# elasota/ConvectionKernels

Measured on AMD Instinct MI355X. Metric: bc7_encode_default_plan_throughput, higher is better.
Workload: dtype f32+u16; 1 GPU; EncodeBC7, BC7EncodingPlan() + Options(), 4096x4096 SplitMix64 random RGBA, seed 2, 1048576 blocks resident in HBM (BASELINE configs[1]); blocks=1048576, exchange=none, search=exact branch-and-bound (output bit-identical)

## Files before the change

### convectionkernels_amd/api.py

```python
import ctypes
import functools
import os
import sys

import numpy as np

_HERE = os.path.dirname(os.path.abspath(__file__))
_LIB_PATH = os.path.join(_HERE, "lib", "libcvtt_mi355x.so")

NumParallelBlocks = 8


class Flags:
    BC7_FastIndexing = 0x008
    BC7_TrySingleColor = 0x010
    BC7_RespectPunchThrough = 0x020
    BC6H_FastIndexing = 0x040
    S3TC_Exhaustive = 0x080
    S3TC_Paranoid = 0x100
    Uniform = 0x200
    ETC_UseFakeBT709 = 0x400
    ETC_FakeBT709Accurate = 0x800
    Fastest = BC6H_FastIndexing | BC7_FastIndexing | S3TC_Paranoid
    Faster = Fastest
# ... 792 lines not shown
            n = b.size // bpb
            if b.size % bpb or n % NumParallelBlocks:
                raise CvttError("packed must hold a multiple of 8 %d-byte blocks" % bpb)
            shape, dt = self._decoded_layout(fmt, n)
            res = np.empty(shape, dt)
            with self._host_lock:
                self._check(self._lib.cvttmi_decode(self._h, fid, res.ctypes.data, b.ctypes.data, n), "decode(%s)" % fmt)
            return res
        import torch
        b = self._device_in(packed, "packed")
        nbytes = b.numel() * b.element_size()
        n = nbytes // bpb
        if nbytes % bpb or n % NumParallelBlocks:
            raise CvttError("packed must hold a multiple of 8 %d-byte blocks" % bpb)
        shape, dt = self._decoded_layout(fmt, n)
        res = torch.empty(shape, dtype={np.int16: torch.int16, np.int8: torch.int8, np.uint8: torch.uint8}[dt], device=b.device)
        stream = self._stream(stream, b.device)
        self._check(self._lib.cvttmi_decode_device(self._h, fid, res.data_ptr(), b.data_ptr(), n, ctypes.c_void_p(stream)),
                    "decode(%s)" % fmt)
        return res

    def measure_error(self, fmt, blocks, packed, per_block=False, stream=None):
        fid, bpb, tex, _ = self._texture_format(fmt)
        hdr = texel_class(fmt) == "half"
        if isinstance(packed, np.ndarray):
            b = np.ascontiguousarray(packed, np.uint8)
            s = np.ascontiguousarray(blocks)
            n = b.size // bpb
            if b.size % bpb or n % NumParallelBlocks or s.nbytes != n * tex:
                raise CvttError("packed must hold a multiple of 8 %d-byte blocks and blocks exactly as many %d-byte source blocks"
                                % (bpb, tex))
            totals = ErrorTotals()
            pb = np.empty(n, np.float32 if hdr else np.uint32) if per_block else None
            with self._host_lock:
                self._check(self._lib.cvttmi_measure_error(self._h, fid, b.ctypes.data, s.ctypes.data, n,
                                                           pb.ctypes.data if per_block else None, ctypes.addressof(totals)),
                            "measure_error(%s)" % fmt)
            return ErrorReport(fmt, totals, pb)
        import torch
        b = self._device_in(packed, "packed")
        s = self._device_in(blocks, "blocks")
        nbytes = b.numel() * b.element_size()
        n = nbytes // bpb
        if nbytes % bpb or n % NumParallelBlocks or s.numel() * s.element_size() != n * tex:
            raise CvttError("packed must hold a multiple of 8 %d-byte blocks and blocks exactly as many %d-byte source blocks"
                            % (bpb, tex))
        return self._measure_device(fmt, n, per_block, stream, b.device, lambda pb, tot, st: self._lib.cvttmi_measure_error_device(
            self._h, fid, b.data_ptr(), s.data_ptr(), n, pb, tot, st))

    def _measure_device(self, fmt, n, per_block, stream, device, call):
        import torch
        hdr = texel_class(fmt) == "half"
        tot = torch.empty(ctypes.sizeof(ErrorTotals), dtype=torch.uint8, device=device)
        pb = torch.empty(n, dtype=torch.float32 if hdr else torch.int32, device=device) if per_block else None
        stream = self._stream(stream, device)
        self._check(call(pb.data_ptr() if per_block else None, tot.data_ptr(), ctypes.c_void_p(stream)), "measure(%s)" % fmt)
        torch.cuda.synchronize(device)
        totals = ErrorTotals.from_buffer_copy(tot.cpu().numpy().tobytes())
        return ErrorReport(fmt, totals, pb)

    def measure_image(self, fmt, image, packed, per_block=False, stream=None):
        import torch
        fid, bpb, _, _ = self._texture_format(fmt)
        if not (isinstance(image, torch.Tensor) and image.is_cuda and image.dim() == 3 and image.shape[2] == 4):
            raise CvttError("image must be a CUDA tensor of shape (H, W, 4)")
        if image.device.index != self.device:
            raise CvttError("image lives on cuda:%d but this context was created for cuda:%d" % (image.device.index, self.device))
        if image.stride(2) != 1 or image.stride(1) != 4:
            image = image.contiguous()
        h, w = int(image.shape[0]), int(image.shape[1])
        esz = image.element_size()
        b = self._device_in(packed, "packed")
        n = ((w + 3) // 4) * ((h + 3) // 4)
        if b.numel() * b.element_size() != n * bpb:
            raise CvttError("packed must hold the %d blocks of a %dx%d image" % (n, w, h))
        return self._measure_device(fmt, n, per_block, stream, b.device, lambda pb, tot, st: self._lib.cvttmi_measure_image_error_device(
            self._h, fid, b.data_ptr(), image.data_ptr(), w, h, image.stride(0) * esz, 0 if esz == 1 else 1, pb, tot, st))

    def selftest_arith(self, count=1 << 22, seed=1):
        d, q = ctypes.c_uint64(0), ctypes.c_uint64(0)
        self._check(self._lib.cvttmi_selftest_arith(self._h, count, seed, ctypes.byref(d), ctypes.byref(q)), "selftest_arith")
        return int(d.value), int(q.value)

    def tile_image(self, image, stream=None):
        import torch
        image = self._image_in(image)
        h, w = int(image.shape[0]), int(image.shape[1])
        esz = image.element_size()
        n = self._lib.cvttmi_tiled_block_count(w, h)
        blocks = torch.empty((n, 16, 4), dtype=image.dtype, device=image.device)
        if stream is None:
            stream = torch.cuda.current_stream(image.device).cuda_stream
        self._check(self._lib.cvttmi_tile_image_device(self._h, blocks.data_ptr(), image.data_ptr(), w, h,
                                                       image.stride(0) * esz, 0 if esz == 1 else 1, ctypes.c_void_p(stream)), "tile_image")
        return blocks

    def compact_rows(self, packed, width, height, stream=None):
        import torch
        packed = self._device_in(packed, "packed")
        bpb = int(packed.shape[1])
        out = torch.empty((((height + 3) // 4) * ((width + 3) // 4), bpb), dtype=torch.uint8, device=packed.device)
        if stream is None:
            stream = torch.cuda.current_stream(packed.device).cuda_stream
        self._check(self._lib.cvttmi_compact_rows_device(self._h, out.data_ptr(), packed.contiguous().data_ptr(), width, height, bpb,
                                                         ctypes.c_void_p(stream)), "compact_rows")
        return out

    def encode_image(self, fmt, image, options=None, plan=None, stream=None):
        h, w = int(image.shape[0]), int(image.shape[1])
        blocks = self.tile_image(image, stream)
        if not has_image_form(fmt):
            raise CvttError("unknown format %r" % (fmt,))
        packed = self.encode(fmt, blocks, options, plan, stream=stream)
        return packed if w % 32 == 0 else self.compact_rows(packed, w, h, stream)

    def _image_in(self, image):
        import torch
        if not (isinstance(image, torch.Tensor) and image.is_cuda and image.dim() == 3 and image.shape[2] == 4):
            raise CvttError("image must be a CUDA tensor of shape (H, W, 4)")
        if image.device.index != self.device:
            raise CvttError("image lives on cuda:%d but this context was created for cuda:%d" % (image.device.index, self.device))
        if image.element_size() not in (1, 2):
            raise CvttError("image must be RGBA8 or RGBA16F")
        return image if image.stride(2) == 1 and image.stride(1) == 4 else image.contiguous()

    def _one_layer(self, image):
        image = self._image_in(image)
        if image.stride(0) < 4 * image.shape[1] or image.stride(0) % 4:
            raise CvttError("image rows must be whole texels and at least a row apart")
        return image[None]

    def build_mips(self, image, levels=None, signed=False, stream=None, filter="box", kernel=None, wrap="clamp"):
        return self.build_mips_array(self._one_layer(image), levels, signed, stream, filter, kernel, wrap)[0]

    def encode_mips(self, fmt, image, options=None, plan=None, levels=None, stream=None, mip_filter="box", kernel=None, wrap="clamp"):
        import torch
        if not has_image_form(fmt):
            raise CvttError("unknown format %r" % (fmt,))
        if isinstance(image, torch.Tensor) and image.dtype == torch.int8 and texel_class(fmt) != "snorm8":
            raise CvttError("%s is not encoded from an int8 image (bc4s / bc5s are)" % fmt)
        return self.encode_texture(fmt, self._one_layer(image), options, plan, levels, "layer", mip_filter, stream, kernel, wrap)[0]

    def _images_in(self, images):
        import torch
        if isinstance(images, (list, tuple)):
            images = [self._image_in(t) for t in images]
            if not images or any(t.shape != images[0].shape or t.dtype != images[0].dtype for t in images):
                raise CvttError("images must be a non-empty list of (H, W, 4) tensors of one size and dtype")
            images = torch.stack(images)
        if not (isinstance(images, torch.Tensor) and images.is_cuda and images.dim() == 4 and images.shape[3] == 4 and images.shape[0] >= 1
                and images.shape[1] >= 1 and images.shape[2] >= 1):
            raise CvttError("images must be a CUDA tensor of shape (L, H, W, 4) or a list of (H, W, 4) CUDA tensors")
        if images.device.index != self.device:
            raise CvttError("images live on cuda:%d but this context was created for cuda:%d" % (images.device.index, self.device))
        if images.element_size() not in (1, 2):
            raise CvttError("images must be RGBA8 or RGBA16F")
        n, h, w = (int(v) for v in images.shape[:3])
        row = images.stride(1) if h > 1 else 4 * w
        layer = images.stride(0) if n > 1 else h * row
        if not (images.stride(3) == 1 and images.stride(2) == 4 and row >= 4 * w and row % 4 == 0 and layer >= h * row and layer % 4 == 0):
            images = images.contiguous()
            row, layer = 4 * w, 4 * w * h
        esz = images.element_size()
        return images, row * esz, layer * esz

    def build_mips_array(self, images, levels=None, signed=False, stream=None, filter="box", kernel=None, wrap="clamp"):
# ... 354 lines not shown
```

### convectionkernels_amd/csrc/bc7_bounds.h

```cpp
#pragma once

namespace
{
typedef short v2s __attribute__((ext_vector_type(2)));

__device__ __forceinline__ int dot2(u32 a, u32 b, int acc)
{
    return __builtin_amdgcn_sdot2(__builtin_bit_cast(v2s, a), __builtin_bit_cast(v2s, b), acc, false);
}

__device__ __forceinline__ constexpr int tri(int r, int c) { return r >= c ? r * (r + 1) / 2 + c : c * (c + 1) / 2 + r; }

struct BlockScatter
{
    float S[10];
    float meanW[4];
};

__device__ __forceinline__ void blockRawSumsQuad(const u32 (&pix)[16], int c, int (&s)[4], int (&p)[10])
{
#pragma unroll
    for (int i = 0; i < 4; i++)
        s[i] = 0;
#pragma unroll
// ... 535 lines not shown
        P.tUU = dot2(P.U[k], P.U[k], P.tUU);
        P.tVV = dot2(P.V[k], P.V[k], P.tVV);
        P.tUV = dot2(P.U[k], P.V[k], P.tUV);
    }
    }
}

struct Sums2D
{
    int n, u, v, uu, vv, uv;
};

__device__ __forceinline__ void maskedSumsSel(const Proj2D<true> &P, int n, const uint4 &sel, Sums2D &m)
{
    m.n = n;
    m.u = m.v = m.uu = m.vv = m.uv = 0;
    const u32 s4[4] = {sel.x, sel.y, sel.z, sel.w};
#pragma unroll
    for (int k = 0; k < 4; k++)
    {
        const u32 um = P.U[k] & s4[k], vm = P.V[k] & s4[k];
        m.u = dot4s(um, 0x01010101u, m.u);
        m.v = dot4s(vm, 0x01010101u, m.v);
        m.uu = dot4s(um, P.U[k], m.uu);
        m.vv = dot4s(vm, P.V[k], m.vv);
        m.uv = dot4s(um, P.V[k], m.uv);
    }
}

template <bool G8>
__device__ __forceinline__ void maskedSums(const Proj2D<G8> &P, u32 mask, Sums2D &m)
{
    m.n = __popc(mask);
    m.u = m.v = m.uu = m.vv = m.uv = 0;
    if constexpr (G8)
    {
#pragma unroll
    for (int k = 0; k < 4; k++)
    {
        const u32 bits = (((mask >> (4 * k)) & 0xfu) * 0x00204081u) & 0x01010101u;
        const u32 sel = (bits << 8) - bits;
        const u32 um = P.U[k] & sel, vm = P.V[k] & sel;
        m.u = dot4s(um, 0x01010101u, m.u);
        m.v = dot4s(vm, 0x01010101u, m.v);
        m.uu = dot4s(um, P.U[k], m.uu);
        m.vv = dot4s(vm, P.V[k], m.vv);
        m.uv = dot4s(um, P.V[k], m.uv);
    }
    }
    else
    {
#pragma unroll
    for (int k = 0; k < 8; k++)
    {
        const u32 lo = (u32)__builtin_amdgcn_sbfe(mask, 2 * k, 1);
        const u32 hi = (u32)__builtin_amdgcn_sbfe(mask, 2 * k + 1, 1);
        const u32 sel = (lo & 0x0000ffffu) | (hi & 0xffff0000u);
        const u32 um = P.U[k] & sel, vm = P.V[k] & sel;
        m.u = dot2(um, 0x00010001u, m.u);
        m.v = dot2(vm, 0x00010001u, m.v);
        m.uu = dot2(um, P.U[k], m.uu);
        m.vv = dot2(vm, P.V[k], m.vv);
        m.uv = dot2(um, P.V[k], m.uv);
    }
    }
}

template <bool G8 = false>
__device__ __forceinline__ float subsetBound2D(const Sums2D &m, float rcpN, float invScaleSq, float twoDelta)
{
    const int a = (G8 ? __mul24(m.n, m.uu) : m.n * m.uu) - __mul24(m.u, m.u);
    const int c = (G8 ? __mul24(m.n, m.vv) : m.n * m.vv) - __mul24(m.v, m.v);
    const int b = (G8 ? __mul24(m.n, m.uv) : m.n * m.uv) - __mul24(m.u, m.v);
    const float fa = (float)a, fc = (float)c, fb = (float)b;
    const float half = (fa + fc) * 0.5f;
    const float diff = (fa - fc) * 0.5f;
    const float rad = __builtin_amdgcn_sqrtf(__fmaf_rn(diff, diff, fb * fb));
    const float lam = half * 0.999998f - rad * 1.000002f;
    const float L = fmaxf(lam, 0.0f) * invScaleSq;
    const float lb = (L * rcpN - twoDelta * __builtin_amdgcn_sqrtf(L)) * 0.9999f;
    return fmaxf(lb, 0.0f);
}

}

__device__ __forceinline__ u32 everyFourth(u64 m, int c)
{
    u64 x = (m >> c) & 0x1111111111111111ull;
    x = (x | (x >> 3)) & 0x0303030303030303ull;
    x = (x | (x >> 6)) & 0x000f000f000f000full;
    x = (x | (x >> 12)) & 0x000000ff000000ffull;
    x = (x | (x >> 24)) & 0xffffull;
    return (u32)x;
}
```

### convectionkernels_amd/csrc/bc7_kernel.hip

```cpp
#include <hip/hip_runtime.h>
#include <stdint.h>
#include <float.h>
#include <type_traits>
#include <stdlib.h>

#include "cvtt_device.h"

constexpr int kMaxPTRefine = 2;
constexpr float kBoundGrid16 = 2000.0f, kBoundLimit16 = 2040.0f;
constexpr float kBoundGrid8 = 124.0f, kBoundLimit8 = 127.0f;
#ifndef CVTT_GRID8_RGBA
#define CVTT_GRID8_RGBA true
#endif
#ifndef CVTT_GRID8_RGB
#define CVTT_GRID8_RGB true
#endif
#ifndef CVTT_BC7_WAVES
#define CVTT_BC7_WAVES 4
#endif
#ifndef CVTT_BC7_WAVES_SLOW
#define CVTT_BC7_WAVES_SLOW 4
#endif
#ifndef CVTT_EIG_ITERS
#define CVTT_EIG_ITERS 6
// ... 41 lines not shown
#define PROF_STAGE_LANES(stage, slot, pred) { const unsigned long long v_ = (unsigned long long)__popcll(__ballot(pred)); if (threadIdx.x == 0 && v_) atomicAdd(&g_bc7Stage[stage][slot], v_); }
#define PROF_STAGE2(stage, slot, n) { const unsigned long long v_ = (unsigned long long)(n); if (threadIdx.x == 0 && v_) atomicAdd(&g_bc7Stage2[stage][slot], v_); }
extern "C" int cvttmi_bc7_dup_read(unsigned long long *out)
{
    unsigned long long zero[8] = {0};
    if (hipMemcpyFromSymbol(out, HIP_SYMBOL(g_bc7Dup), sizeof(zero)) != hipSuccess) return -1;
    if (hipMemcpyToSymbol(HIP_SYMBOL(g_bc7Dup), zero, sizeof(zero)) != hipSuccess) return -1;
    return 0;
}
#define PROF_DECL unsigned long long profT = __builtin_readcyclecounter(); unsigned long long profAcc[16] = {0, 0, 0, 0, 0, 0, 0, 0, 0, 0, 0, 0, 0, 0, 0, 0}; unsigned long long profCnt[8] = {0, 0, 0, 0, 0, 0, 0, 0};
#define PROF_MARK(slot) { const unsigned long long now = __builtin_readcyclecounter(); profAcc[slot] += now - profT; profT = now; }
#define PROF_FLUSH if (threadIdx.x == 0) { unsigned long long tot = 0; for (int i = 0; i < 16; i++) { atomicAdd(&g_bc7Prof[i], profAcc[i]); tot += profAcc[i]; } \
    int bucket = 63 - __builtin_clzll(tot | 1ull) - 12; bucket = bucket < 0 ? 0 : (bucket > 15 ? 15 : bucket); atomicAdd(&g_bc7Prof[16 + bucket], 1ull); \
    } { unsigned long long wsum[8]; for (int i = 0; i < 8; i++) { unsigned long long v = profCnt[i]; if (i >= 4) { for (int st = 1; st < 64; st <<= 1) v += __shfl_xor(v, st); } wsum[i] = v; } \
    if (threadIdx.x == 0) { for (int i = 0; i < 8; i++) atomicAdd(&g_bc7Prof[32 + i], wsum[i]); \
    const unsigned long long passes = profCnt[2] / 64ull; int pb = 63 - __builtin_clzll(passes | 1ull); pb = pb > 7 ? 7 : pb; atomicAdd(&g_bc7Prof[40 + pb], 1ull); } }
#define PROF_COUNT(slot, n) { profCnt[slot] += (unsigned long long)(n); }
extern "C" int cvttmi_bc7_prof_read(unsigned long long *out)
{
    unsigned long long zero[48] = {0};
    if (hipMemcpyFromSymbol(out, HIP_SYMBOL(g_bc7Prof), sizeof(zero)) != hipSuccess) return -1;
    if (hipMemcpyToSymbol(HIP_SYMBOL(g_bc7Prof), zero, sizeof(zero)) != hipSuccess) return -1;
    return 0;
}
#else
#define PROF_DECL
#define PROF_MARK(slot)
#define PROF_COUNT(slot, n)
#define PROF_FLUSH
#define PROF_STAGE(stage, slot, n)
#define PROF_STAGE2(stage, slot, n)
#define PROF_STAGE_LANES(stage, slot, pred)
#endif

#ifdef CVTT_BC7_BOUND_DUMP
__device__ u32 *g_bc7BoundBuf;
__device__ u32 g_bc7BoundCap;
__device__ u32 g_bc7BoundCount;
extern "C" int cvttmi_bc7_bound_dump_set(void *deviceBuffer, uint32_t capacityRecords)
{
    const uint32_t zero = 0;
    u32 *buf = static_cast<u32 *>(deviceBuffer);
    if (hipMemcpyToSymbol(HIP_SYMBOL(g_bc7BoundBuf), &buf, sizeof(buf)) != hipSuccess) return -1;
    if (hipMemcpyToSymbol(HIP_SYMBOL(g_bc7BoundCap), &capacityRecords, sizeof(capacityRecords)) != hipSuccess) return -1;
    if (hipMemcpyToSymbol(HIP_SYMBOL(g_bc7BoundCount), &zero, sizeof(zero)) != hipSuccess) return -1;
    return 0;
}
extern "C" int cvttmi_bc7_bound_dump_count(uint32_t *out)
{
    return hipMemcpyFromSymbol(out, HIP_SYMBOL(g_bc7BoundCount), sizeof(*out)) == hipSuccess ? 0 : -1;
}
enum : u32 { BD_WHOLE6 = 0, BD_ROT = 1, BD_TIER1 = 2, BD_FULL = 3, BD_SHARP = 4, BD_PROBE_FULL = 5, BD_PROBE_SHARP = 6, BD_FINAL = 7 };
enum : u32 { BD_FORM = 0, BD_FORM_CMP = 1, BD_RELOAD = 2, BD_SUBSET = 3, BD_END = 4 };
__device__ __noinline__ void boundDumpEmit(u32 block, u32 w1, u32 w2, u32 w3, float computed, float stored, float err, u32 dropped,
                                           float x0, float x1, float x2, float x3)
{
    u32 *const buf = g_bc7BoundBuf;
    if (buf == nullptr)
        return;
    const u32 at = atomicAdd(&g_bc7BoundCount, 1u);
    if (at >= g_bc7BoundCap)
        return;
    u32 *r = buf + (size_t)at * 12u;
    r[0] = block;
    r[1] = w1;
    r[2] = w2;
    r[3] = w3;
    r[4] = __builtin_bit_cast(u32, computed);
    r[5] = __builtin_bit_cast(u32, stored);
    r[6] = __builtin_bit_cast(u32, err);
    r[7] = dropped;
    r[8] = __builtin_bit_cast(u32, x0);
    r[9] = __builtin_bit_cast(u32, x1);
    r[10] = __builtin_bit_cast(u32, x2);
    r[11] = __builtin_bit_cast(u32, x3);
}
#define BOUND_DUMP(...) do { __VA_ARGS__; } while (0)
#else
#define BOUND_DUMP(...)
#endif

#include "bc7_chain.h"
#include "bc7_dual.h"
#include "bc7_bounds.h"

template <bool FAST, bool PT, bool HARD>
__device__ __forceinline__ void bc7Body(const uint8_t *__restrict__ blocks, uint8_t *__restrict__ out,
                                        const CvttBc7Args &A, const CvttDeviceTables *__restrict__ T,
                                        const CvttBc7DevicePlan *__restrict__ dplan, const u32 vBlock, const u32 vGrid)
{
    __shared__ unsigned short s_bound[64][16];
    auto lbLoadRaw = [&](int partition, int b) -> float { return __builtin_bit_cast(float, (u32)s_bound[partition][b] << 16); };
    auto lbLoad = [&](int partition, int b) -> float { return __builtin_fabsf(lbLoadRaw(partition, b)); };
    auto lbStore = [&](int partition, int b, float v) { s_bound[partition][b] = (unsigned short)(__builtin_bit_cast(u32, v) >> 16); };
    auto lbStoreTier2 = [&](int partition, int b, float v) { s_bound[partition][b] = (unsigned short)((__builtin_bit_cast(u32, v) >> 16) | 0x8000u); };
    u32 *const s_raw = reinterpret_cast<u32 *>(&s_bound[0][0]);
    __shared__ u32 s_pix[16][16];
    __shared__ u32 s_blkFlags[16];
    __shared__ int s_scatter[16][14];
    __shared__ u32 s_item[64];
    __shared__ uint8_t s_myItems[PT ? 16 : 1][32];
    __shared__ UnitRec s_unit[64];
    __shared__ u32 s_parked[16][2];
    __shared__ float s_static[16];
    __shared__ unsigned short s_pm2[64];
    __shared__ u32 s_pm3[64];
    __shared__ __attribute__((aligned(16))) u32 s_res[64][5];
    __shared__ float s_trialErr[PT ? 32 * 16 * kMaxPTRefine : 1];
    float *const trialHbm = (PT && A.ptTrial) ? A.ptTrial + (size_t)vBlock * (size_t)(32 * 16) * (size_t)(A.refineRounds < 1 ? 1 : A.refineRounds) : nullptr;
    const cvttmi_bc7_plan *__restrict__ plan = &dplan->plan;
    int lane = threadIdx.x;
    int c = lane & 3;
    int blk = lane >> 2;
#define REFRESH_LANE() do { lane = (int)__builtin_amdgcn_mbcnt_hi(~0u, __builtin_amdgcn_mbcnt_lo(~0u, 0u)); asm volatile("" : "+v"(lane)); c = lane & 3; blk = lane >> 2; } while (0)
    u32 hardIndex = 0, hardBlock = 0;
    u64 hardMine = 0;
    float hardErr = FLT_MAX;
    int hardSeq = -1;
    if (HARD)
    {
        hardIndex = vBlock / kHardWaves;
        const u32 count = *A.hardCount;
        if (hardIndex >= (count < A.hardCap ? count : A.hardCap))
            return;
        const CvttBc7HardRec rec = A.hardRec[hardIndex];
        hardBlock = rec.blockIndex;
        hardErr = rec.err;
        hardSeq = rec.seq;
        u64 m = ((u64)rec.aliveHi << 32) | rec.aliveLo;
        const int q = (int)(vBlock % kHardWaves);
        for (int r = 0; m != 0; r++)
        {
            const u64 low = m & (0ull - m);
            if ((r % kHardWaves) == q)
                hardMine |= low;
            m ^= low;
        }
        if (hardMine == 0)
        {
            if (lane == 0)
                A.hardCand[vBlock].err = FLT_MAX;
            return;
        }
    }
    const u32 blockIndex = (HARD ? (hardBlock & ~15u) : vBlock * 16u) + (u32)(lane >> 2);
    const bool inRange = blockIndex < A.numBlocks;
#ifdef CVTT_BC7_BOUND_DUMP
    auto bdEmit = [&](u32 tier, u32 kind, u32 set, u32 mode, u32 numSub, u32 bits, u32 part, u32 sub, float computed, float stored, float err,
                      bool dropped, float x0 = 0.0f, float x1 = 0.0f, float x2 = 0.0f, float x3 = 0.0f) {
        boundDumpEmit(blockIndex, tier | (kind << 8) | (HARD ? 1u << 16 : 0u), set | (mode << 8) | (numSub << 16) | (bits << 24), part | (sub << 8),
                      computed, stored, err, dropped ? 1u : 0u, x0, x1, x2, x3);
    };
#endif
    enum : u32 { LF_VALID = 1u, LF_ANY_ALPHA = 2u, LF_ALLOW_RGB = 4u, LF_ALLOW_M7 = 8u, LF_NONMAX_ALPHA = 16u };
    u32 lf = (inRange && (!HARD || blockIndex == hardBlock)) ? LF_VALID : 0u;
#define valid ((lf & LF_VALID) != 0)
#define anyBlockHasAlpha ((lf & LF_ANY_ALPHA) != 0)
#define allowRGBModes ((lf & LF_ALLOW_RGB) != 0)
#define allowMode7 ((lf & LF_ALLOW_M7) != 0)
#define blockHasNonMaxAlpha ((lf & LF_NONMAX_ALPHA) != 0)

    PROF_DECL
    s_pm2[lane] = T->partition2[lane];
    s_pm3[lane] = (u32)T->subsetMask3[lane][0] | ((u32)T->subsetMask3[lane][1] << 16);
    __syncthreads();
    u32 pix[16];
// ... 418 lines not shown
    {
        REFRESH_LANE();
        const int stageIter = (ballotA == 0 && !HARD) ? ((stageOrder == 1) ? 2 : (stageOrder == 2) ? 3 : (stageOrder == 3) ? 1 : stageOrder) : stageOrder;
        ModeDesc md;
        int numSubsets, numPartitions, stage, boundSet;
        switch (stageIter)
        {
        case 0: stage = 4; md = {6, 4, 4, 7, 0}; numSubsets = 1; numPartitions = 1; boundSet = 3; break;
        case 1: stage = 5; md = {7, 2, 4, 5, 6}; numSubsets = 2; numPartitions = 64; boundSet = 0; break;
        case 2: stage = 1; md = {1, 3, 2, 6, 7}; numSubsets = 2; numPartitions = 64; boundSet = 1; break;
        case 3: stage = 3; md = {3, 2, 4, 7, 0}; numSubsets = 2; numPartitions = 64; boundSet = 1; break;
        case 4: stage = 0; md = {0, 3, 4, 4, 5}; numSubsets = 3; numPartitions = 16; boundSet = 2; break;
        default: stage = 2; md = {2, 2, 1, 5, 5}; numSubsets = 3; numPartitions = 64; boundSet = 2; break;
        }
        if (HARD && stageIter != 1)
            continue;
        if (stageIter == 1 && ballotA == 0)
            boundSet = 1;
        const int mode = md.mode;
        const bool isRGB = mode < 4;
        const bool laneRuns = isRGB ? allowRGBModes : (mode == 7 ? allowMode7 : true);
        if (__ballot(laneRuns) == 0)
            continue;
        u64 enabled;
        switch (stageIter)
        {
        case 0: enabled = plan->mode6Enabled ? 1 : 0; break;
        case 1: enabled = ~0ull; break;
        case 2: enabled = plan->mode1PartitionEnabled; break;
        case 3: enabled = plan->mode3PartitionEnabled; break;
        case 4: enabled = plan->mode0PartitionEnabled & 0xffffull; break;
        default: enabled = plan->mode2PartitionEnabled; break;
        }
        if (HARD)
            enabled = hardMine;
        if (enabled == 0)
            continue;

        u32 freshAlive = 0;
        bool freshBounds = false;
        if (prune)
        {
            if (WS_GET(WS_BOUNDS_FOR) == boundSet + 1 && WS_GET(WS_BOUND_BITS) < md.indexBits)
                WS_SET(WS_BOUNDS_FOR, 0);
            if (WS_GET(WS_BOUNDS_FOR) != boundSet + 1)
            {
                WS_SET(WS_BOUND_BITS, 4);
                WS_SET(WS_SHARP_RAN, 4);
                __syncthreads();
                if (boundSet == 3)
                {
                }
                else
                {
                    const bool use4 = (boundSet == 0);
                    auto boundsOnGrid = [&](auto g8) {
                    constexpr bool G8 = decltype(g8)::value;
                    const float wsum = A.wSqSum3 + (use4 ? A.wSq[3] : 0.0f);
                    const float scale = (G8 ? kBoundGrid8 : kBoundGrid16) / (255.0f * __builtin_amdgcn_sqrtf(wsum));
                    const float invScaleSq = 1.0f / (scale * scale);
                    const float twoDelta = 2.0f * ((use4 ? A.delta4 : A.delta3) + 0.7072f / scale);
                    const float staticErr = use4 ? 0.0f : s_static[blk];
                    const int rcpLane = (int)kRcpDown[lane < 16 ? lane : 16];
                    auto rcpOf = [&](int n) -> float { return __builtin_bit_cast(float, __builtin_amdgcn_ds_bpermute(n << 2, rcpLane)); };
                    Proj2D<G8> P;
                    PROF_MARK(2)
                    {
                        BlockScatter bsL;
                        {
                            int rs[4], rp[10];
#pragma unroll
                            for (int i = 0; i < 10; i++)
                                rp[i] = s_scatter[blk][i];
#pragma unroll
                            for (int i = 0; i < 4; i++)
                                rs[i] = s_scatter[blk][10 + i];
                            scatterFromRaw(rs, rp, A, bsL);
                        }
                        u32 lpix[16];
                        pixFromLds(lpix);
                        makeProjection(lpix, bsL, A, use4, scale, P);
                    }
                    PROF_MARK(7)
                    const bool two = boundSet < 2;
                    auto selOf = [&](int partition, int which) -> uint4 {
                        return *reinterpret_cast<const uint4 *>(T->subsetByteMask[two ? partition : 64 + 2 * partition + which]);
                    };
                    uint4 selA = make_uint4(0, 0, 0, 0), selB = make_uint4(0, 0, 0, 0);
                    if constexpr (G8)
                    {
                        selA = selOf(c, 0);
                        if (!two)
                            selB = selOf(c, 1);
                    }
                    for (int k = 0; k < 16; k++)
                    {
                        const int partition = 4 * k + c;
                        float lb;
                        uint4 selA1 = selA, selB1 = selB;
                        if constexpr (G8)
                        {
                            const int nextPartition = (k < 15 ? partition + 4 : partition);
                            selA1 = selOf(nextPartition, 0);
                            if (!two)
                                selB1 = selOf(nextPartition, 1);
                        }
                        if (boundSet < 2)
                        {
                            Sums2D s1, s0;
                            if constexpr (G8)
                                maskedSumsSel(P, __popc((u32)s_pm2[partition]), selA, s1);
                            else
                                maskedSums(P, s_pm2[partition], s1);
                            s0.n = 16 - s1.n;
                            s0.u = P.tU - s1.u;
                            s0.v = P.tV - s1.v;
                            s0.uu = P.tUU - s1.uu;
                            s0.vv = P.tVV - s1.vv;
                            s0.uv = P.tUV - s1.uv;
                            lb = subsetBound2D<G8>(s0, rcpOf(s0.n), invScaleSq, twoDelta) + subsetBound2D<G8>(s1, rcpOf(s1.n), invScaleSq, twoDelta);
                        }
                        else
                        {
                            Sums2D s1, s2, s0;
                            if constexpr (G8)
                            {
                                maskedSumsSel(P, __popc(s_pm3[partition] & 0xffffu), selA, s1);
                                maskedSumsSel(P, __popc(s_pm3[partition] >> 16), selB, s2);
                            }
                            else
                            {
                            maskedSums(P, s_pm3[partition] & 0xffffu, s1);
                            maskedSums(P, s_pm3[partition] >> 16, s2);
                            }
                            s0.n = 16 - s1.n - s2.n;
                            s0.u = P.tU - s1.u - s2.u;
                            s0.v = P.tV - s1.v - s2.v;
                            s0.uu = P.tUU - s1.uu - s2.uu;
                            s0.vv = P.tVV - s1.vv - s2.vv;
                            s0.uv = P.tUV - s1.uv - s2.uv;
                            lb = subsetBound2D<G8>(s0, rcpOf(s0.n), invScaleSq, twoDelta) + subsetBound2D<G8>(s1, rcpOf(s1.n), invScaleSq, twoDelta) +
                                 subsetBound2D<G8>(s2, rcpOf(s2.n), invScaleSq, twoDelta);
                        }
                        lb += staticErr;
                        lbStore(partition, blk, lb);
                        BOUND_DUMP(if (valid) bdEmit(BD_TIER1, BD_FORM_CMP, (u32)boundSet, (u32)mode, (u32)numSubsets, 4, (u32)partition, 0, lb, lbLoad(partition, blk),
                                                     work.err, lb > work.err, staticErr));
                        freshAlive |= (lb > work.err) ? 0u : (1u << k);
                        selA = selA1;
                        selB = selB1;
                    }
                    freshBounds = true;
                    };
                    if (use4 ? CVTT_GRID8_RGBA : CVTT_GRID8_RGB)
                        boundsOnGrid(std::true_type{});
                    else
                        boundsOnGrid(std::false_type{});
                }
                __syncthreads();
                WS_SET(WS_BOUNDS_FOR, boundSet + 1);
            }
        }
        PROF_MARK(2)

        const int CP = md.numP * 4;
        const int UPB = 64 / CP;
        u32 aliveBits = (valid && laneRuns) ? everyFourth(enabled, c) : 0u;
        if (mode == 7 && anyBlockHasAlpha && !blockHasNonMaxAlpha)
            aliveBits &= everyFourth(mode7RGB, c);
        u32 tier2Done = 0;
        if (prune)
        {
            if (freshBounds)
                aliveBits &= freshAlive;
            else
            {
                for (int k = 0; k * 4 < numPartitions; k++)
                {
                    const float raw = lbLoadRaw(4 * k + c, blk);
                    BOUND_DUMP(if ((aliveBits >> k) & 1u) bdEmit(boundSet == 3 ? BD_WHOLE6 : (__builtin_bit_cast(u32, raw) >> 31) ? (WS_GET(WS_SHARP_RAN) < 4 ? BD_SHARP : BD_FULL) : BD_TIER1,
                                                                 BD_RELOAD, (u32)boundSet, (u32)mode, (u32)numSubsets, (u32)md.indexBits, (u32)(4 * k + c), 0,
                                                                 __builtin_fabsf(raw), __builtin_fabsf(raw), work.err, __builtin_fabsf(raw) > work.err, (float)WS_GET(WS_BOUND_BITS)));
                    if (__builtin_fabsf(raw) > work.err)
                        aliveBits &= ~(1u << k);
                    tier2Done |= (__builtin_bit_cast(u32, raw) >> 31) << k;
                }
            }
        }

        if (prune && numSubsets >= 2)
// ... 1380 lines not shown
```

### convectionkernels_amd/csrc/selftest_kernel.hip

```cpp
#include "cvtt_kernel_common.h"

namespace
{
__device__ __forceinline__ u64 mix64(u64 z)
{
    z = (z ^ (z >> 30)) * 0xBF58476D1CE4E5B9ull;
    z = (z ^ (z >> 27)) * 0x94D049BB133111EBull;
    return z ^ (z >> 31);
}

__global__ void cvttmi_selftest_kernel(u64 seed, u64 first, u32 count, u32 *__restrict__ operands, u32 *__restrict__ results)
{
    const u32 i = blockIdx.x * blockDim.x + threadIdx.x;
    if (i >= count)
        return;
    const u64 r = mix64(seed + (first + i) * 0x9E3779B97F4A7C15ull);
    u32 a = (u32)r, b = (u32)(r >> 32);
    if ((a & 0x7f800000u) == 0x7f800000u) a ^= 0x00800000u;
    if ((b & 0x7f800000u) == 0x7f800000u) b ^= 0x00800000u;
    const float fa = __uint_as_float(a), fb = __uint_as_float(b);
    operands[2 * i] = a;
    operands[2 * i + 1] = b;
    results[2 * i] = __float_as_uint(fa / fb);
    results[2 * i + 1] = __float_as_uint(sqrtExact(__uint_as_float(a & 0x7fffffffu)));
}
}

extern "C" hipError_t cvttmi_launch_selftest(uint64_t seed, uint64_t first, uint32_t count, void *d_operands, void *d_results,
                                             hipStream_t stream)
{
    if (count == 0)
        return hipSuccess;
    hipLaunchKernelGGL(cvttmi_selftest_kernel, dim3((count + 255u) / 256u), dim3(256), 0, stream, seed, first, count,
                       (u32 *)d_operands, (u32 *)d_results);
    return hipGetLastError();
}
```

### convectionkernels_amd/csrc/shim.cpp

```cpp
#include <hip/hip_runtime.h>

#include <stdio.h>
#include <stddef.h>
#include <stdlib.h>
#include <string.h>
#include <vector>
#include <utility>
#include <xmmintrin.h>
#include <math.h>

#include <mutex>
#include <string>

#include "cvtt_device.h"
#include "source_id.h"
#include "bc7_tables.h"
#include "s3tc_sc_tables.h"
#include "bc7_quality_events.h"
#include "fake709_rounding.h"
#include "bc6h_layout.h"
#include "etc_tables.h"
#include "texture_formats.h"
#include "srgb_tables.h"
#include "mip_kernel_tables.h"

extern "C" hipError_t cvttmi_launch_bc7(const void *d_blocks, void *d_out, const CvttBc7Args *args,
                                        const CvttDeviceTables *d_tables, const CvttBc7DevicePlan *d_plan,
                                        hipStream_t stream);

extern "C" hipError_t cvttmi_launch_tile(const void *d_image, void *d_blocks, uint32_t width, uint32_t height, size_t rowPitch,
                                         uint32_t bytesPerPixel, hipStream_t stream);
extern "C" hipError_t cvttmi_launch_compact_rows(const void *d_packed, void *d_out, uint32_t width, uint32_t height,
                                                 uint32_t bytesPerBlock, hipStream_t stream);
extern "C" hipError_t cvttmi_launch_downsample(const void *d_src, size_t srcPitch, size_t srcLayer, void *d_dst, size_t dstPitch,
                                               size_t dstLayer, uint32_t srcW, uint32_t srcH, uint32_t layers, int kind, hipStream_t stream);
extern "C" hipError_t cvttmi_launch_downsample_filtered(const void *d_src, size_t srcPitch, size_t srcLayer, void *d_dst, size_t dstPitch,
                                                        size_t dstLayer, uint32_t srcW, uint32_t srcH, uint32_t layers, int kind,
                                                        uint32_t filter, hipStream_t stream);
extern "C" hipError_t cvttmi_launch_resample(const void *d_src, size_t srcPitch, size_t srcLayer, void *d_dst, size_t dstPitch, size_t dstLayer,
                                             uint32_t srcW, uint32_t srcH, uint32_t layers, int kind, uint32_t rule, uint32_t wrap,
                                             const int16_t *taps, uint32_t count, hipStream_t stream);
extern "C" size_t cvttmi_resize_entry_bytes(uint32_t rule);
extern "C" uint32_t cvttmi_resize_fused_rows(uint32_t rule, const int32_t *first, uint32_t dstH, uint32_t ny);
extern "C" hipError_t cvttmi_launch_resize(const void *d_src, size_t srcPitch, size_t srcLayer, uint32_t srcW, uint32_t srcH, void *d_dst,
                                           size_t dstPitch, size_t dstLayer, uint32_t dstW, uint32_t dstH, uint32_t layers, int kind,
                                           uint32_t rule, uint32_t wrap, const int16_t *d_wx, const int32_t *d_fx, uint32_t nx,
                                           const int16_t *d_wy, const int32_t *d_fy, uint32_t ny, void *d_mid, uint32_t fusedRows,
                                           hipStream_t stream);
extern "C" hipError_t cvttmi_launch_tile_chain(const CvttTextureLevels *levels, void *d_tiles, uint32_t bytesPerPixel, hipStream_t stream);
extern "C" hipError_t cvttmi_launch_compact_chain(const CvttTextureLevels *levels, const void *d_packed, void *d_out, uint32_t bytesPerBlock,
                                                  hipStream_t stream);
extern "C" hipError_t cvttmi_launch_selftest(uint64_t seed, uint64_t first, uint32_t count, void *d_operands, void *d_results,
                                             hipStream_t stream);
extern "C" hipError_t cvttmi_launch_decode(const void *d_bc, void *d_out, uint32_t numBlocks, int format, const CvttDeviceTables *d_tables,
                                           hipStream_t stream);
extern "C" hipError_t cvttmi_launch_measure(const void *d_bc, const void *d_source, int source, uint32_t width, uint32_t height,
                                            size_t pitch, size_t firstBlock, uint32_t numBlocks, int format, void *d_blockError, void *d_slab,
                                            cvttmi_error_totals *d_totals, int accumulate, uint64_t texels,
                                            const CvttDeviceTables *d_tables, hipStream_t stream);
extern "C" hipError_t cvttmi_launch_decode_image(const void *d_bc, void *d_image, size_t pitch, uint32_t width, uint32_t height, int format,
                                                 const CvttDeviceTables *d_tables, hipStream_t stream);
extern "C" hipError_t cvttmi_launch_decode_mips(const void *d_bc, const CvttDecodeLevels *levels, int format, const CvttDeviceTables *d_tables,
                                                hipStream_t stream);
extern "C" hipError_t cvttmi_launch_eac11(const void *d_blocksS16, void *d_out, uint32_t numBlocks, int isSigned,
                                          const CvttDeviceTables *d_tables, hipStream_t stream);
extern "C" hipError_t cvttmi_launch_s3tc_alpha(const void *d_blocks, void *d_out, uint32_t numBlocks, uint32_t channel, uint32_t outStride,
                                               uint32_t outOffset, int isSigned, int explicitAlpha, int seedPoints, int refineRounds,
                                               const CvttDeviceTables *d_tables, hipStream_t stream);
extern "C" hipError_t cvttmi_launch_bc1(const void *d_blocks, void *d_out, const CvttBc1Args *args,
                                        const CvttDeviceTables *d_tables, hipStream_t stream);

extern "C" hipError_t cvttmi_launch_bc6h(const void *d_blocks, void *d_out, const CvttBc6hArgs *args,
                                         const CvttDeviceTables *d_tables, int isSigned, hipStream_t stream);

extern "C" hipError_t cvttmi_launch_etc2(const void *d_blocks, void *d_out, const CvttEtcArgs *args,
                                         const CvttDeviceTables *d_tables, int mode, hipStream_t stream);

static_assert(sizeof(cvttmi_options) == 44, "cvtt::Options layout");
static_assert(sizeof(cvttmi_bc7_plan) == 808, "cvtt::BC7EncodingPlan layout");
static_assert(sizeof(cvttmi_error_totals) == 80 && offsetof(cvttmi_error_totals, sseHdr) == 32 &&
              offsetof(cvttmi_error_totals, texels) == 64 && offsetof(cvttmi_error_totals, channelMask) == 72 &&
              offsetof(cvttmi_error_totals, format) == 76, "cvttmi_error_totals layout");

struct cvttmi_context
{
    int device;
    CvttDeviceTables hostTables;
    CvttDeviceTables *dTables;
    static const int kPlanSlots = 8;
    CvttBc7DevicePlan *dPlans;
    CvttBc7DevicePlan *pinnedPlans;
    cvttmi_bc7_plan lastPlan[kPlanSlots];
    bool planValid[kPlanSlots];
    static const int kPlanUsers = 4;
    struct PlanUse
    {
        hipStream_t stream;
        hipEvent_t ev;
        bool valid;
    } planUse[kPlanSlots][kPlanUsers];
    hipEvent_t evPlanUp[kPlanSlots];
    hipStream_t planUpStream[kPlanSlots];
    int nextPlanSlot;
    static const int kPipeSlots = 4;
    struct PipeSlot
    {
        void *pinnedIn, *pinnedOut, *dIn, *dOut;
        hipStream_t stream;
        hipEvent_t done;
    } pipe[kPipeSlots];
    size_t pipeInBytes, pipeOutBytes;
    hipStream_t stream;
    std::recursive_mutex mu;
    hipEvent_t evLast;
    hipStream_t lastStream;
    bool lastValid;
    float *dPtTrial;
    size_t dPtTrialBytes;
    size_t ptTableBytes;
    bool exhaustive;
    void *dMeasureSlab = NULL;
    void *dMeasureHost = NULL;
    size_t measureHostBytes = 0;
    static const int kResizeSlots = 4;
    struct ResizeSlot
    {
        void *pinned = NULL;
        size_t bytes = 0;
        hipEvent_t ev = NULL;
        hipStream_t stream = NULL;
        bool inFlight = false, valid = false;
        uint32_t srcW = 0, srcH = 0, dstW = 0, dstH = 0, filter = 0;
    } resizeSlot[kResizeSlots];
    int nextResizeSlot = 0;
// ... 2142 lines not shown
            });
        });
    }

    double cvttmi_psnr(const cvttmi_error_totals *t, uint32_t channelMask)
    {
        uint32_t fmask = 0;
        const CvttTextureFormat *row = t ? formatInfo(t->format, NULL, NULL, &fmask) : NULL;
        if (!row || row->peak == 0)
            return NAN;
        const uint32_t m = channelMask ? channelMask : fmask;
        if ((m & ~fmask) != 0 || t->texels == 0)
            return NAN;
        uint64_t sse = 0;
        int channels = 0;
        for (int c = 0; c < 4; c++)
            if ((m >> c) & 1u)
            {
                sse += t->sse[c];
                channels++;
            }
        if (sse == 0)
            return INFINITY;
        const double peak = row->peak;
        const double mse = static_cast<double>(sse) / (static_cast<double>(t->texels) * channels);
        return 10.0 * log10(peak * peak / mse);
    }

    int cvttmi_selftest_arith(cvttmi_context *ctx, uint64_t count, uint64_t seed, uint64_t *divMismatches, uint64_t *sqrtMismatches)
    {
        if (!ctx || !divMismatches || !sqrtMismatches)
            return CVTTMI_E_INVALID;
        hipError_t e = hipSetDevice(ctx->device);
        if (e != hipSuccess)
            return fail(ctx, CVTTMI_E_NO_DEVICE, "hipSetDevice", e);
        const uint32_t chunk = 1u << 20;
        uint32_t *dOps = NULL, *dRes = NULL;
        if (hipMalloc(&dOps, chunk * 8) != hipSuccess || hipMalloc(&dRes, chunk * 8) != hipSuccess)
        {
            hipFree(dOps);
            return fail(ctx, CVTTMI_E_HIP, "hipMalloc (selftest)");
        }
        std::vector<uint32_t> ops(chunk * 2), res(chunk * 2);
        uint64_t badDiv = 0, badSqrt = 0;
        for (uint64_t first = 0; first < count; first += chunk)
        {
            const uint32_t n = static_cast<uint32_t>(count - first < chunk ? count - first : chunk);
            e = cvttmi_launch_selftest(seed, first, n, dOps, dRes, NULL);
            if (e == hipSuccess) e = hipMemcpy(ops.data(), dOps, (size_t)n * 8, hipMemcpyDeviceToHost);
            if (e == hipSuccess) e = hipMemcpy(res.data(), dRes, (size_t)n * 8, hipMemcpyDeviceToHost);
            if (e != hipSuccess)
            {
                hipFree(dOps);
                hipFree(dRes);
                return fail(ctx, CVTTMI_E_HIP, "selftest kernel", e);
            }
            for (uint32_t i = 0; i < n; i++)
            {
                float a, b;
                memcpy(&a, &ops[2 * i], 4);
                memcpy(&b, &ops[2 * i + 1], 4);
                const float q = _mm_cvtss_f32(_mm_div_ss(_mm_set_ss(a), _mm_set_ss(b)));
                uint32_t absBits = ops[2 * i] & 0x7fffffffu;
                float absA;
                memcpy(&absA, &absBits, 4);
                const float r = _mm_cvtss_f32(_mm_sqrt_ss(_mm_set_ss(absA)));
                uint32_t qb, rb;
                memcpy(&qb, &q, 4);
                memcpy(&rb, &r, 4);
                const bool qNan = (qb & 0x7fffffffu) > 0x7f800000u, gNan = (res[2 * i] & 0x7fffffffu) > 0x7f800000u;
                if (!(qNan && gNan) && qb != res[2 * i])
                    badDiv++;
                if (rb != res[2 * i + 1])
                    badSqrt++;
            }
        }
        hipFree(dOps);
        hipFree(dRes);
        *divMismatches = badDiv;
        *sqrtMismatches = badSqrt;
        return CVTTMI_OK;
    }

    int cvttmi_set_exhaustive(cvttmi_context *ctx, int exhaustive)
    {
        if (!ctx)
            return CVTTMI_E_INVALID;
        ctx->exhaustive = exhaustive != 0;
        return CVTTMI_OK;
    }

    int cvttmi_bc7_hard_stats(cvttmi_context *ctx, uint32_t *handedOver, uint32_t *slots)
    {
        if (!ctx)
            return CVTTMI_E_INVALID;
        hipSetDevice(ctx->device);
        hipDeviceSynchronize();
        if (ctx->handOver.stats(handedOver, slots) != hipSuccess)
            return fail(ctx, CVTTMI_E_HIP, "hipMemcpy(hard count)");
        return CVTTMI_OK;
    }

    int cvttmi_timing_enable(cvttmi_context *ctx, int enable)
    {
        if (!ctx)
            return CVTTMI_E_INVALID;
        ctx->timing = enable != 0;
        ctx->totalMs = 0.0;
        ctx->launches = 0;
        return CVTTMI_OK;
    }

    int cvttmi_timing_read(cvttmi_context *ctx, double *totalMs, uint64_t *launches)
    {
        if (!ctx)
            return CVTTMI_E_INVALID;
        if (totalMs) *totalMs = ctx->totalMs;
        if (launches) *launches = ctx->launches;
        return CVTTMI_OK;
    }

    int cvttmi_format_info(int format, size_t *packedBytes, size_t *blockBytes, uint32_t *channelMask)
    { return formatInfo(format, packedBytes, blockBytes, channelMask) ? CVTTMI_OK : CVTTMI_E_INVALID; }

    int cvttmi_encode_device(cvttmi_context *ctx, int format, void *d_out, const void *d_blocks, size_t numBlocks,
                             const cvttmi_options *options, const cvttmi_bc7_plan *plan, const cvttmi_options *allocOptions, void *hipStream)
    {
        size_t packedBytes = 16, blockBytes = 64;
        const bool ok = formatInfo(format, &packedBytes, &blockBytes, NULL) && options && (plan || !kEncoderFormats[format].takesPlan);
        return onDevice(ctx, d_out, d_blocks, numBlocks, ok, blockBytes, packedBytes, hipStream, encodeBody(ctx, format, options, plan, allocOptions));
    }
    int cvttmi_encode(cvttmi_context *ctx, int format, void *out, const void *blocks, size_t numBlocks,
                      const cvttmi_options *options, const cvttmi_bc7_plan *plan, const cvttmi_options *allocOptions)
    {
        size_t packedBytes = 16, blockBytes = 64;
        const bool known = formatInfo(format, &packedBytes, &blockBytes, NULL);
        const bool ok = known && options && (plan || !kEncoderFormats[format].takesPlan);
        return onHost(ctx, out, blocks, numBlocks, ok, blockBytes, packedBytes, known && kEncoderFormats[format].zeroCopy,
                      encodeBody(ctx, format, options, plan, allocOptions));
    }

    int cvttmi_encode_bc7_device(cvttmi_context *ctx, void *d_out, const void *d_blocks, size_t numBlocks,
                                 const cvttmi_options *options, const cvttmi_bc7_plan *plan, void *hipStream)
    { return cvttmi_encode_device(ctx, CVTTMI_FMT_BC7, d_out, d_blocks, numBlocks, options, plan, NULL, hipStream); }
    int cvttmi_encode_bc7(cvttmi_context *ctx, uint8_t *out, const uint8_t *blocks, size_t numBlocks,
                          const cvttmi_options *options, const cvttmi_bc7_plan *plan)
    { return cvttmi_encode(ctx, CVTTMI_FMT_BC7, out, blocks, numBlocks, options, plan, NULL); }

    static int etc2KindFormat(int kind)
    {
        return kind == CVTTMI_ETC2_RGB ? CVTTMI_FMT_ETC2_RGB : kind == CVTTMI_ETC2_RGBA ? CVTTMI_FMT_ETC2_RGBA
             : kind == CVTTMI_ETC2_PUNCHTHROUGH ? CVTTMI_FMT_ETC2_PUNCHTHROUGH : -1;
    }
    int cvttmi_encode_etc2_with_data_device(cvttmi_context *ctx, void *d_out, const void *d_blocks, size_t numBlocks, const cvttmi_options *options,
                                            const cvttmi_options *allocOptions, int kind, void *hipStream)
    { return cvttmi_encode_device(ctx, etc2KindFormat(kind), d_out, d_blocks, numBlocks, options, NULL, allocOptions, hipStream); }
    int cvttmi_encode_etc2_with_data(cvttmi_context *ctx, uint8_t *out, const uint8_t *blocks, size_t numBlocks, const cvttmi_options *options,
                                     const cvttmi_options *allocOptions, int kind)
    { return cvttmi_encode(ctx, etc2KindFormat(kind), out, blocks, numBlocks, options, NULL, allocOptions); }

    int cvttmi_encode_etc2_device(cvttmi_context *ctx, void *d_out, const void *d_blocks, size_t numBlocks, const cvttmi_options *options, void *hipStream)
    { return cvttmi_encode_device(ctx, CVTTMI_FMT_ETC2_RGB, d_out, d_blocks, numBlocks, options, NULL, NULL, hipStream); }
    int cvttmi_encode_etc2_rgba_device(cvttmi_context *ctx, void *d_out, const void *d_blocks, size_t numBlocks, const cvttmi_options *options, void *hipStream)
    { return cvttmi_encode_device(ctx, CVTTMI_FMT_ETC2_RGBA, d_out, d_blocks, numBlocks, options, NULL, NULL, hipStream); }
    int cvttmi_encode_etc2_alpha_device(cvttmi_context *ctx, void *d_out, const void *d_blocks, size_t numBlocks, const cvttmi_options *options, void *hipStream)
    { return cvttmi_encode_device(ctx, CVTTMI_FMT_EAC_ALPHA, d_out, d_blocks, numBlocks, options, NULL, NULL, hipStream); }
// ... 54 lines not shown
```

Measured before the change: 726.0 Mblocks/s.

## Compute tier-1 two-subset partition sums with int8 MFMA matrix multiply

For the G8 grid path with two-subset bound sets, per-block projected feature sums across all 64 partitions are now computed as an int8 32x32x16 MFMA between feature operands and partition-mask operands, instead of per-partition scalar accumulation. The complement subset sums come from stored block totals. Lower bounds are then evaluated and alive masks are gathered via ballot into shared memory. This adds shared-memory staging and two extra barriers, and relies on the quadratic terms being split into 7-bit pieces to fit int8 exactly. An MFMA self-test entry point is also added.

```diff
diff --git a/convectionkernels_amd/api.py b/convectionkernels_amd/api.py
--- a/convectionkernels_amd/api.py
+++ b/convectionkernels_amd/api.py
@@ -898,6 +898,17 @@
         self._check(self._lib.cvttmi_selftest_arith(self._h, count, seed, ctypes.byref(d), ctypes.byref(q)), "selftest_arith")
         return int(d.value), int(q.value)
 
+    def selftest_mfma_i8(self, a, b):
+        a = np.ascontiguousarray(a, dtype=np.int8)
+        b = np.ascontiguousarray(b, dtype=np.int8)
+        if a.shape != (32, 16) or b.shape != (16, 32):
+            raise CvttError("selftest_mfma_i8 takes a (32, 16) and a (16, 32) int8 array")
+        out = np.empty((32, 32), np.int32)
+        fn = self._lib.cvttmi_selftest_mfma_i8
+        fn.argtypes = [ctypes.c_void_p, ctypes.c_void_p, ctypes.c_void_p, ctypes.c_void_p]
+        self._check(fn(self._h, a.ctypes.data, b.ctypes.data, out.ctypes.data), "selftest_mfma_i8")
+        return out
+
     def tile_image(self, image, stream=None):
         import torch
         image = self._image_in(image)
diff --git a/convectionkernels_amd/csrc/bc7_bounds.h b/convectionkernels_amd/csrc/bc7_bounds.h
--- a/convectionkernels_amd/csrc/bc7_bounds.h
+++ b/convectionkernels_amd/csrc/bc7_bounds.h
@@ -641,6 +641,44 @@
     return fmaxf(lb, 0.0f);
 }
 
+constexpr int kT1RecWords = 16;
+constexpr int kT1AliveAt = 16 * kT1RecWords;
+
+__device__ __forceinline__ constexpr int t1RowQuantity(int r) { return (r & 3) + 4 * ((r >> 3) & 1); }
+__device__ __forceinline__ constexpr int t1RowBlock(int r) { return 2 * (r >> 4) + ((r >> 2) & 1); }
+
+__device__ __forceinline__ u64 t1MaskOperand(u32 mask16, int h)
+{
+    const u32 m8 = (mask16 >> (8 * h)) & 0xffu;
+    const u32 lo = ((m8 & 0xfu) * 0x00204081u) & 0x01010101u;
+    const u32 hi = ((m8 >> 4) * 0x00204081u) & 0x01010101u;
+    return (u64)lo | ((u64)hi << 32);
+}
+
+__device__ __forceinline__ u64 t1FeatureOperand(const u32 *rec, int h, int q)
+{
+    const uint2 U = *reinterpret_cast<const uint2 *>(rec + 2 * h), V = *reinterpret_cast<const uint2 *>(rec + 4 + 2 * h);
+    const bool firstV = (q == 1) | (q == 4) | (q == 5), secondU = (q == 2) | (q == 3);
+    const u32 a[2] = {firstV ? V.x : U.x, firstV ? V.y : U.y};
+    const u32 b[2] = {secondU ? U.x : V.x, secondU ? U.y : V.y};
+    const int sh = (q & 1) ? 7 : 0;
+    const u32 keep = (q & 1) ? 0xffu : 0x7fu;
+    u32 w[2];
+#pragma unroll
+    for (int i = 0; i < 2; i++)
+    {
+        u32 acc = 0;
+#pragma unroll
+        for (int k = 0; k < 4; k++)
+        {
+            const int x = __builtin_amdgcn_sbfe((int)a[i], 8 * k, 8), y = __builtin_amdgcn_sbfe((int)b[i], 8 * k, 8);
+            acc |= ((u32)(__mul24(x, y) >> sh) & keep) << (8 * k);
+        }
+        w[i] = (q < 2) ? a[i] : acc;
+    }
+    return (u64)w[0] | ((u64)w[1] << 32);
+}
+
 }
 
 __device__ __forceinline__ u32 everyFourth(u64 m, int c)
diff --git a/convectionkernels_amd/csrc/bc7_kernel.hip b/convectionkernels_amd/csrc/bc7_kernel.hip
--- a/convectionkernels_amd/csrc/bc7_kernel.hip
+++ b/convectionkernels_amd/csrc/bc7_kernel.hip
@@ -147,6 +147,7 @@
 
 #include "bc7_chain.h"
 #include "bc7_dual.h"
+#include "mfma_i8.h"
 #include "bc7_bounds.h"
 
 template <bool FAST, bool PT, bool HARD>
@@ -731,7 +732,86 @@
                         makeProjection(lpix, bsL, A, use4, scale, P);
                     }
                     PROF_MARK(7)
-                    const bool two = boundSet < 2;
+                    bool byMatrix = false;
+                    if constexpr (G8)
+                        byMatrix = boundSet < 2;
+                    if constexpr (G8)
+                    if (byMatrix)
+                    {
+                        u32 *const s_t1 = &s_res[0][0];
+                        if (c == 0)
+                        {
+                            uint4 *const rec = reinterpret_cast<uint4 *>(s_t1 + blk * kT1RecWords);
+                            rec[0] = make_uint4(P.U[0], P.U[1], P.U[2], P.U[3]);
+                            rec[1] = make_uint4(P.V[0], P.V[1], P.V[2], P.V[3]);
+                            rec[2] = make_uint4((u32)P.tU, (u32)P.tV, (u32)P.tUU, (u32)P.tVV);
+                            rec[3] = make_uint4((u32)P.tUV, __builtin_bit_cast(u32, work.err), __builtin_bit_cast(u32, staticErr), 0u);
+                        }
+                        __syncthreads();
+                        const int h = lane >> 5;
+                        u64 maskOp[2];
+                        int n1[2];
+                        float rcp1[2], rcp0[2];
+#pragma unroll
+                        for (int t = 0; t < 2; t++)
+                        {
+                            const u32 m = s_pm2[(lane & 31) + 32 * t];
+                            maskOp[t] = t1MaskOperand(m, h);
+                            n1[t] = __popc(m);
+                            rcp1[t] = __builtin_bit_cast(float, kRcpDown[n1[t]]);
+                            rcp0[t] = __builtin_bit_cast(float, kRcpDown[16 - n1[t]]);
+                        }
+                        const int rowQ = t1RowQuantity(lane & 31);
+                        const u32 *const featRec = s_t1 + t1RowBlock(lane & 31) * kT1RecWords;
+#pragma unroll 1
+                        for (int g = 0; g < 4; g++)
+                        {
+                            const u64 featOp = t1FeatureOperand(featRec + 4 * g * kT1RecWords, h, rowQ);
+#pragma unroll
+                            for (int t = 0; t < 2; t++)
+                            {
+                                const v16i zero = {0, 0, 0, 0, 0, 0, 0, 0, 0, 0, 0, 0, 0, 0, 0, 0};
+                                const v16i acc = mfmaI8(featOp, maskOp[t], zero);
+                                const int partition = (lane & 31) + 32 * t;
+#pragma unroll
+                                for (int j = 0; j < 2; j++)
+                                {
+                                    const int block = 4 * g + 2 * j + h;
+                                    const uint4 tot = *reinterpret_cast<const uint4 *>(s_t1 + block * kT1RecWords + 8);
+                                    const uint4 tail = *reinterpret_cast<const uint4 *>(s_t1 + block * kT1RecWords + 12);
+                                    Sums2D s1, s0;
+                                    s1.n = n1[t];
+                                    s1.u = acc[8 * j + 0];
+                                    s1.v = acc[8 * j + 1];
+                                    s1.uu = acc[8 * j + 2] + (int)((u32)acc[8 * j + 3] << 7);
+                                    s1.vv = acc[8 * j + 4] + (int)((u32)acc[8 * j + 5] << 7);
+                                    s1.uv = acc[8 * j + 6] + (int)((u32)acc[8 * j + 7] << 7);
+                                    s0.n = 16 - s1.n;
+                                    s0.u = (int)tot.x - s1.u;
+                                    s0.v = (int)tot.y - s1.v;
+                                    s0.uu = (int)tot.z - s1.uu;
+                                    s0.vv = (int)tot.w - s1.vv;
+                                    s0.uv = (int)tail.x - s1.uv;
+                                    const float blockErr = __builtin_bit_cast(float, tail.y);
+                                    float lb = subsetBound2D<true>(s0, rcp0[t], invScaleSq, twoDelta) + subsetBound2D<true>(s1, rcp1[t], invScaleSq, twoDelta);
+                                    lb += __builtin_bit_cast(float, tail.z);
+                                    lbStore(partition, block, lb);
+                                    BOUND_DUMP(if (vBlock * 16u + (u32)block < A.numBlocks)
+                                                   boundDumpEmit(vBlock * 16u + (u32)block, BD_TIER1 | (BD_FORM_CMP << 8), (u32)boundSet | ((u32)mode << 8) | ((u32)numSubsets << 16) | (4u << 24),
+                                                                 (u32)partition, lb, lbLoad(partition, block), blockErr, lb > blockErr ? 1u : 0u,
+                                                                 __builtin_bit_cast(float, tail.z), 0.0f, 0.0f, 0.0f));
+                                    const u64 stay = __ballot(!(lb > blockErr));
+                                    if (lane == 0)
+                                        *reinterpret_cast<uint2 *>(s_t1 + kT1AliveAt + 16 * t + 4 * g + 2 * j) = make_uint2((u32)stay, (u32)(stay >> 32));
+                                }
+                            }
+                        }
+                        __syncthreads();
+                        freshAlive = everyFourth((u64)s_t1[kT1AliveAt + blk] | ((u64)s_t1[kT1AliveAt + 16 + blk] << 32), c);
+                        freshBounds = true;
+                        return;
+                    }
+                    const bool two = !G8 && boundSet < 2;
                     auto selOf = [&](int partition, int which) -> uint4 {
                         return *reinterpret_cast<const uint4 *>(T->subsetByteMask[two ? partition : 64 + 2 * partition + which]);
                     };
@@ -754,7 +834,7 @@
                             if (!two)
                                 selB1 = selOf(nextPartition, 1);
                         }
-                        if (boundSet < 2)
+                        if (two)
                         {
                             Sums2D s1, s0;
                             if constexpr (G8)
diff --git a/convectionkernels_amd/csrc/mfma_i8.h b/convectionkernels_amd/csrc/mfma_i8.h
--- /dev/null
+++ b/convectionkernels_amd/csrc/mfma_i8.h
@@ -0,0 +1,11 @@
+#pragma once
+#include "cvtt_kernel_common.h"
+
+typedef int v16i __attribute__((ext_vector_type(16)));
+
+__device__ __forceinline__ v16i mfmaI8(u64 a, u64 b, v16i c)
+{
+    return __builtin_amdgcn_mfma_i32_32x32x16_i8((long)a, (long)b, c, 0, 0, 0);
+}
+
+__device__ __forceinline__ constexpr int mfmaRowOf(int reg, int laneHalf) { return (reg & 3) + 8 * (reg >> 2) + 4 * laneHalf; }
diff --git a/convectionkernels_amd/csrc/selftest_kernel.hip b/convectionkernels_amd/csrc/selftest_kernel.hip
--- a/convectionkernels_amd/csrc/selftest_kernel.hip
+++ b/convectionkernels_amd/csrc/selftest_kernel.hip
@@ -1,4 +1,5 @@
 #include "cvtt_kernel_common.h"
+#include "mfma_i8.h"
 
 namespace
 {
@@ -24,6 +25,29 @@
     results[2 * i] = __float_as_uint(fa / fb);
     results[2 * i + 1] = __float_as_uint(sqrtExact(__uint_as_float(a & 0x7fffffffu)));
 }
+
+__global__ void cvttmi_selftest_mfma_i8_kernel(const int8_t *__restrict__ a, const int8_t *__restrict__ b, int *__restrict__ out)
+{
+    const int l = threadIdx.x, rc = l & 31, kh = l >> 5;
+    u64 av = 0, bv = 0;
+#pragma unroll
+    for (int t = 0; t < 8; t++)
+    {
+        av |= (u64)(uint8_t)a[rc * 16 + 8 * kh + t] << (8 * t);
+        bv |= (u64)(uint8_t)b[(8 * kh + t) * 32 + rc] << (8 * t);
+    }
+    v16i acc = {0, 0, 0, 0, 0, 0, 0, 0, 0, 0, 0, 0, 0, 0, 0, 0};
+    acc = mfmaI8(av, bv, acc);
+#pragma unroll
+    for (int r = 0; r < 16; r++)
+        out[mfmaRowOf(r, kh) * 32 + rc] = acc[r];
+}
+}
+
+extern "C" hipError_t cvttmi_launch_selftest_mfma_i8(const void *d_a, const void *d_b, void *d_out, hipStream_t stream)
+{
+    hipLaunchKernelGGL(cvttmi_selftest_mfma_i8_kernel, dim3(1), dim3(64), 0, stream, (const int8_t *)d_a, (const int8_t *)d_b, (int *)d_out);
+    return hipGetLastError();
 }
 
 extern "C" hipError_t cvttmi_launch_selftest(uint64_t seed, uint64_t first, uint32_t count, void *d_operands, void *d_results,
diff --git a/convectionkernels_amd/csrc/shim.cpp b/convectionkernels_amd/csrc/shim.cpp
--- a/convectionkernels_amd/csrc/shim.cpp
+++ b/convectionkernels_amd/csrc/shim.cpp
@@ -50,6 +50,7 @@
 extern "C" hipError_t cvttmi_launch_tile_chain(const CvttTextureLevels *levels, void *d_tiles, uint32_t bytesPerPixel, hipStream_t stream);
 extern "C" hipError_t cvttmi_launch_compact_chain(const CvttTextureLevels *levels, const void *d_packed, void *d_out, uint32_t bytesPerBlock,
                                                   hipStream_t stream);
+extern "C" hipError_t cvttmi_launch_selftest_mfma_i8(const void *d_a, const void *d_b, void *d_out, hipStream_t stream);
 extern "C" hipError_t cvttmi_launch_selftest(uint64_t seed, uint64_t first, uint32_t count, void *d_operands, void *d_results,
                                              hipStream_t stream);
 extern "C" hipError_t cvttmi_launch_decode(const void *d_bc, void *d_out, uint32_t numBlocks, int format, const CvttDeviceTables *d_tables,
@@ -2358,6 +2359,26 @@
         return CVTTMI_OK;
     }
 
+    int cvttmi_selftest_mfma_i8(cvttmi_context *ctx, const int8_t *a, const int8_t *b, int32_t *out)
+    {
+        if (!ctx || !a || !b || !out)
+            return CVTTMI_E_INVALID;
+        hipError_t e = hipSetDevice(ctx->device);
+        if (e != hipSuccess)
+            return fail(ctx, CVTTMI_E_NO_DEVICE, "hipSetDevice", e);
+        char *d = NULL;
+        if (hipMalloc(&d, 512 + 512 + 4096) != hipSuccess)
+            return fail(ctx, CVTTMI_E_HIP, "hipMalloc (selftest)");
+        e = hipMemcpy(d, a, 512, hipMemcpyHostToDevice);
+        if (e == hipSuccess) e = hipMemcpy(d + 512, b, 512, hipMemcpyHostToDevice);
+        if (e == hipSuccess) e = cvttmi_launch_selftest_mfma_i8(d, d + 512, d + 1024, NULL);
+        if (e == hipSuccess) e = hipMemcpy(out, d + 1024, 4096, hipMemcpyDeviceToHost);
+        hipFree(d);
+        if (e != hipSuccess)
+            return fail(ctx, CVTTMI_E_HIP, "selftest (mfma i8) kernel", e);
+        return CVTTMI_OK;
+    }
+
     int cvttmi_set_exhaustive(cvttmi_context *ctx, int exhaustive)
     {
         if (!ctx)
```

After: 748.1 Mblocks/s (median of 6 runs). +3.0%, better.
